# MGI-tech-bioinformatics/SuperPlus

Hardware: AMD Instinct MI355X
Metric: k-mers/s (DF createDict stage: trim + canonical k-mer count + solid filter + spectrum + adjacency) (higher is better)
Workload: dtype u64

## Files before the change

superplus_amd/csrc/dfk.hip:

```cpp
#include "../../include/dfk.h"
#include "dfk_kernels.h"

#include <algorithm>
#include <chrono>
#include <cstdarg>
#include <cstdio>
#include <cstdlib>
#include <cstring>
#include <atomic>
#include <fcntl.h>
#include <functional>
#include <new>
#include <string>
#include <sys/mman.h>
#include <sys/stat.h>
#include <unistd.h>
#include <condition_variable>
#include <memory>
#include <mutex>
#include <thread>
#include <vector>

using namespace dfk;

// ... 271 lines not shown
    float stop() { (void)hipEventRecord(b, s); (void)hipEventSynchronize(b); float ms = 0; (void)hipEventElapsedTime(&ms, a, b); return ms; }
};

uint32_t ceil_log2(uint64_t v) { uint32_t b = 0; while ((1ull << b) < v) ++b; return b; }

template <int K>
int stage_trim(dfk_ctx* c, const Inputs& in, uint64_t* n_inst)
{
    DevBuf ctr; int rc = c->alloc(ctr, 32, "trim counters"); if (rc) return rc;
    HIP_TRY(hipMemsetAsync(ctr.p, 0, 32, c->stream));
    rc = c->alloc(c->good_len, sizeof(uint32_t) * in.n_reads, "goodLens", true); if (rc) return rc;
    if (in.n_reads) {
        unsigned grid = (unsigned)std::min<uint64_t>((in.n_reads + 255) / 256, 8192);
        hipLaunchKernelGGL(HIP_KERNEL_NAME(k_trim<K>), dim3(grid), dim3(256), 0, c->stream,
                           in.pq, in.pq_off, in.pq_bytes, in.base_off, in.packed_bytes, in.read_len, in.n_reads, c->cfg.min_qual, (uint32_t*)c->good_len.p,
                           (unsigned long long*)ctr.p, (unsigned int*)((char*)ctr.p + 8),
                           (unsigned long long*)((char*)ctr.p + 16));
        HIP_TRY(hipGetLastError());
    }
    uint64_t h[3] = {0, 0, 0};
    HIP_TRY(hipMemcpyAsync(h, ctr.p, 24, hipMemcpyDeviceToHost, c->stream));
    HIP_TRY(hipStreamSynchronize(c->stream));
    c->release(ctr);
    if ((uint32_t)h[1]) return fail(DFK_E_INPUT, "malformed input: an offset table is not monotone or runs past its array, a PQVec stream is broken, or its length differs from read_len");
    if (h[2] == 0) return fail(DFK_E_NOGOOD, "Looks like your input data have almost no good bases.");
    *n_inst = h[0];
    return 0;
}

int device_scan(dfk_ctx* c, const uint64_t* in, uint64_t* out, uint64_t n)
{
    constexpr uint64_t PER = (uint64_t)SCAN_THREADS * SCAN_ITEMS;
    if (n == 0) return 0;
    const uint64_t nblk = (n + PER - 1) / PER;
    if (nblk == 1) {
        hipLaunchKernelGGL(k_scan_blocks, dim3(1), dim3(SCAN_THREADS), 0, c->stream, in, out, n, (uint64_t*)nullptr);
        HIP_TRY(hipGetLastError());
        return 0;
    }
    DevBuf sums; int rc = c->alloc(sums, nblk * 8, "scan block sums"); if (rc) return rc;
    hipLaunchKernelGGL(k_scan_blocks, dim3((unsigned)nblk), dim3(SCAN_THREADS), 0, c->stream, in, out, n, (uint64_t*)sums.p);
    HIP_TRY(hipGetLastError());
    rc = device_scan(c, (const uint64_t*)sums.p, (uint64_t*)sums.p, nblk); if (rc) return rc;
    hipLaunchKernelGGL(k_scan_add, dim3((unsigned)nblk), dim3(SCAN_THREADS), 0, c->stream, out, n, (const uint64_t*)sums.p);
    HIP_TRY(hipGetLastError());
    HIP_TRY(hipStreamSynchronize(c->stream));
    c->release(sums);
    return 0;
}

struct BucketTable {
    uint32_t log2_nb = 0;
    DevBuf acc;
    DevBuf summ;
    DevBuf classes;
    DevBuf ovf_list; uint64_t n_ovf = 0;
    DevBuf class_hist;
    std::vector<uint64_t> h_class;
    uint64_t n_records = 0, n_inst = 0;
};
struct Partition {
    DevBuf records, base, ipre, items;
    uint64_t n_records = 0, n_inst = 0, n_items = 0;
    uint64_t nb = 0;
};

template <int K>
PartParams part_params(const dfk_ctx* c, uint32_t log2_nb, uint32_t log2_world, int64_t read_id0, uint32_t sub_lo, uint32_t sub_n)
{
    const uint32_t M = c->cfg.minimizer_len;
    return PartParams{M, (uint32_t)K - M + 1, log2_nb, log2_world, read_id0, sub_lo, sub_n,
                      sweep_class_mask(sub_lo, sub_n, log2_nb - log2_world)};
}

int table_totals(dfk_ctx* c, const DevBuf& acc, uint64_t nb, uint64_t* n_records, uint64_t* n_inst)
{
    DevBuf tot; int rc = c->alloc(tot, 16, "bucket totals"); if (rc) return rc;
    HIP_TRY(hipMemsetAsync(tot.p, 0, 16, c->stream));
    hipLaunchKernelGGL(k_sum_acc, dim3(1024), dim3(256), 0, c->stream, (const unsigned long long*)acc.p, nb, (unsigned long long*)tot.p);
    HIP_TRY(hipGetLastError());
    uint64_t h[2];
    HIP_TRY(hipMemcpyAsync(h, tot.p, 16, hipMemcpyDeviceToHost, c->stream));
    HIP_TRY(hipStreamSynchronize(c->stream));
    c->release(tot);
    *n_records = h[0]; *n_inst = h[1];
    return 0;
}

struct ScanJob {
    PartParams pp; uint64_t nb = 0, n_bins = 0, ovf_cap = 0; bool by_class = false, ranged = false;
    DevBuf ovf_tmp, d_n;
    bool keyed = false; uint32_t n_cls = 0, n_sub = 0, sb = 0; uint64_t piece_reads = 0;
    ScanKeys sk{};
    DevBuf keys, keys2, fill, sub;
    std::vector<std::pair<hipEvent_t, hipEvent_t>> ev;
    ~ScanJob() { for (auto& e : ev) { (void)hipEventDestroy(e.first); (void)hipEventDestroy(e.second); } }
};

template <int K> bool scan_takes_ranges(const dfk_ctx* c) { return c->cfg.minimizer_len == 16; }

template <int K>
int scan_begin(dfk_ctx* c, const Inputs& in, uint32_t log2_world, int64_t read_id0, BucketTable* T, bool by_class, ScanJob* J)
{
    J->pp = part_params<K>(c, T->log2_nb, log2_world, read_id0, 0, 1u << (T->log2_nb - log2_world));
    J->nb = 1ull << T->log2_nb; J->by_class = by_class;
    int rc = 0;
    J->n_bins = 2ull * (PART_CLASSES << log2_world);
    if (by_class) { rc = c->alloc(T->class_hist, J->n_bins * 8, "class counters", true); if (rc) return rc; HIP_TRY(hipMemsetAsync(T->class_hist.p, 0, J->n_bins * 8, c->stream)); }
    else { rc = c->alloc(T->acc, J->nb * 8, "bucket counters", true); if (rc) return rc; }
    rc = c->alloc(T->summ, std::max<uint64_t>(1, in.n_reads) * 16, "run summaries", true); if (rc) return rc;
    rc = c->alloc(T->classes, std::max<uint64_t>(1, in.n_reads) * 4, "read bucket classes", true); if (rc) return rc;
    if (!by_class) HIP_TRY(hipMemsetAsync(T->acc.p, 0, J->nb * 8, c->stream));
    J->ovf_cap = in.n_reads / 16 + 1024;
    rc = c->alloc(J->ovf_tmp, J->ovf_cap * 4, "overflow read list (scratch)"); if (rc) return rc;
    rc = c->alloc(J->d_n, 16, "overflow read count"); if (rc) return rc;
    HIP_TRY(hipMemsetAsync(J->d_n.p, 0, 16, c->stream));
    const double runs = in.n_reads ? 1.0 + 2.0 * std::max(0.0, 4.0 * (double)in.packed_bytes / (double)in.n_reads - K + 1) / (J->pp.W + 1) : 0.0;
    J->keyed = !by_class && scan_takes_ranges<K>(c) && in.n_reads && (runs >= 3.5 || getenv("DFK_SCAN_KEY_PIECE"));
    if (J->keyed) {
        const uint32_t lb = T->log2_nb, cb = std::min<uint32_t>(6, lb);
        J->sk.ib = lb - cb; J->n_cls = 1u << cb;
        J->sb = std::min(KEY_SUB_BITS, J->sk.ib); J->n_sub = 1u << (J->sk.ib - J->sb);
        const double per_read = 1.25 * runs;
        constexpr uint64_t KEY_SCRATCH_MAX = 16ull << 30;
        const uint64_t want = 8ull * (uint64_t)(per_read * (double)in.n_reads) + 8ull * J->n_cls;
        const uint64_t room = std::min<uint64_t>(std::min(want, KEY_SCRATCH_MAX), c->largest_allocatable() / 3);
        J->sk.cap = std::max<uint64_t>(1024, room / 8 / J->n_cls);
        J->piece_reads = std::max<uint64_t>(PART_THREADS, (uint64_t)((double)(J->sk.cap * J->n_cls) / per_read));
        if (const char* e = getenv("DFK_SCAN_KEY_PIECE")) J->piece_reads = std::max<uint64_t>(1, std::min<uint64_t>(J->piece_reads, strtoull(e, nullptr, 10)));
        const uint64_t n_subs = (uint64_t)J->n_cls * J->n_sub;
        rc = c->alloc(J->keys, J->sk.cap * J->n_cls * 4, "run keys (scratch)"); if (rc) return rc;
        rc = c->alloc(J->keys2, J->sk.cap * J->n_cls * 4, "run keys by sub-slice (scratch)"); if (rc) return rc;
        rc = c->alloc(J->fill, J->n_cls * 8, "run key slice fills (scratch)"); if (rc) return rc;
        rc = c->alloc(J->sub, (3 * n_subs + 1) * 8, "run key sub-slices (scratch)"); if (rc) return rc;
        J->sk.keys = (uint32_t*)J->keys.p; J->sk.fill = (unsigned long long*)J->fill.p;
        TRACE("run keys: %u classes of %llu keys, %u sub-slices each, pieces of %llu reads", J->n_cls, (unsigned long long)J->sk.cap,
              J->n_sub, (unsigned long long)J->piece_reads);
    }
    return 0;
}

template <int K>
int scan_keys_piece(dfk_ctx* c, const Inputs& in, BucketTable* T, ScanJob* J, uint64_t r0, uint64_t r1)
{
    static const unsigned scan_blocks = getenv("DFK_SCAN_BLOCKS") ? (unsigned)atoi(getenv("DFK_SCAN_BLOCKS")) : 0;
    const unsigned cus = (unsigned)c->prop.multiProcessorCount;
    const unsigned grid = (unsigned)std::min<uint64_t>((r1 - r0 + PART_THREADS - 1) / PART_THREADS, (uint64_t)(scan_blocks ? scan_blocks : 128u) * cus);
    const uint64_t n_subs = (uint64_t)J->n_cls * J->n_sub;
    auto* cnt = (unsigned long long*)J->sub.p;
    auto* off = cnt + n_subs;
    auto* cur = off + n_subs + 1;
    HIP_TRY(hipMemsetAsync(J->fill.p, 0, J->n_cls * 8, c->stream));
    HIP_TRY(hipMemsetAsync(cnt, 0, n_subs * 8, c->stream));
    const size_t lds = sizeof(uint32_t) * (PART_RING + SUMMARY_RUNS) * PART_THREADS + SCAN_STAGE_LDS;
    hipLaunchKernelGGL(HIP_KERNEL_NAME(k_scan_count<K, 16, true>), dim3(grid), dim3(PART_THREADS), lds, c->stream,
                       in.packed, in.packed_bytes, in.base_off, (const uint32_t*)c->good_len.p, r0, r1, J->pp,
                       (unsigned long long*)T->acc.p, (unsigned long long*)nullptr, (unsigned long long*)J->d_n.p, J->ovf_cap,
                       (uint32_t*)J->ovf_tmp.p, (uint4*)T->summ.p, (uint32_t*)T->classes.p, J->sk);
    HIP_TRY(hipGetLastError());
    const dim3 per_class(std::max(1u, 16u * cus / J->n_cls), J->n_cls);
    const uint32_t sh = 6 + J->sb;
    hipLaunchKernelGGL(k_keys_subcount, per_class, dim3(256), J->n_sub * 4, c->stream,
                       (const uint32_t*)J->keys.p, (const unsigned long long*)J->fill.p, J->sk.cap, sh, J->n_sub, cnt);
    HIP_TRY(hipGetLastError());
    hipLaunchKernelGGL(k_keys_offsets, dim3(1), dim3(1024), 0, c->stream, (const unsigned long long*)cnt, (uint32_t)n_subs, off, cur);
    HIP_TRY(hipGetLastError());
    hipLaunchKernelGGL(k_keys_partition, per_class, dim3(256), J->n_sub * 12, c->stream,
                       (const uint32_t*)J->keys.p, (const unsigned long long*)J->fill.p, J->sk.cap, sh, J->n_sub, cur, (uint32_t*)J->keys2.p);
    HIP_TRY(hipGetLastError());
    hipLaunchKernelGGL(k_keys_count, dim3((unsigned)n_subs), dim3(1024), 0, c->stream,
                       (const uint32_t*)J->keys2.p, (const unsigned long long*)off, J->sb, (unsigned long long*)T->acc.p);
    HIP_TRY(hipGetLastError());
    return 0;
}

template <int K>
int scan_range(dfk_ctx* c, const Inputs& in, BucketTable* T, ScanJob* J, uint64_t r0, uint64_t r1)
{
    if (r1 <= r0) return 0;
    const PartParams& pp = J->pp;
    const bool by_class = J->by_class;
    unsigned grid = (unsigned)((r1 - r0 + PART_THREADS - 1) / PART_THREADS);
    static const unsigned scan_blocks = getenv("DFK_SCAN_BLOCKS") ? (unsigned)atoi(getenv("DFK_SCAN_BLOCKS")) : 0;
    if (by_class) grid = std::min<unsigned>(grid, (scan_blocks ? scan_blocks : 128u) * (unsigned)c->prop.multiProcessorCount);
    else if (scan_blocks) grid = std::min<unsigned>(grid, scan_blocks * (unsigned)c->prop.multiProcessorCount);
    const size_t lds_a = (sizeof(uint32_t) + 1) * pp.W * PART_THREADS + sizeof(uint32_t) * PART_RING * PART_THREADS + (by_class ? J->n_bins * 4 : 0);
    hipEvent_t e0, e1;
    HIP_TRY(hipEventCreate(&e0)); HIP_TRY(hipEventCreate(&e1));
    J->ev.emplace_back(e0, e1);
    HIP_TRY(hipEventRecord(e0, c->stream));
    if (J->keyed) {
        for (uint64_t p0 = r0; p0 < r1; p0 += J->piece_reads) {
            int rc = scan_keys_piece<K>(c, in, T, J, p0, std::min(r1, p0 + J->piece_reads)); if (rc) return rc;
        }
    } else if (scan_takes_ranges<K>(c)) {
        const size_t lds_r = sizeof(uint32_t) * (PART_RING + SUMMARY_RUNS) * PART_THREADS + (by_class ? J->n_bins * 4 : 0);
        hipLaunchKernelGGL(HIP_KERNEL_NAME(k_scan_count<K, 16, false>), dim3(grid), dim3(PART_THREADS), lds_r, c->stream,
                           in.packed, in.packed_bytes, in.base_off, (const uint32_t*)c->good_len.p, r0, r1, pp,
                           (unsigned long long*)T->acc.p, (unsigned long long*)T->class_hist.p, (unsigned long long*)J->d_n.p, J->ovf_cap,
                           (uint32_t*)J->ovf_tmp.p, (uint4*)T->summ.p, (uint32_t*)T->classes.p, ScanKeys{});
    } else {
        if (r0 != 0 || r1 != in.n_reads) return fail(DFK_E_STATE, "the general scan takes every read at once");
        hipLaunchKernelGGL(HIP_KERNEL_NAME(k_partition<K, false>), dim3(grid), dim3(PART_THREADS), lds_a, c->stream,
                           in.packed, in.packed_bytes, in.base_off, (const uint32_t*)c->good_len.p, in.bc,
                           (int64_t)c->cfg.ign_bc_below, in.n_reads, pp, (unsigned long long*)T->acc.p, (unsigned long long*)T->class_hist.p,
                           (unsigned long long*)J->d_n.p, J->ovf_cap, (uint4*)J->ovf_tmp.p, (uint4*)T->summ.p,
                           (const uint32_t*)nullptr, (uint64_t)0, (const uint64_t*)nullptr, (uint32_t*)T->classes.p);
    }
    HIP_TRY(hipGetLastError());
    HIP_TRY(hipEventRecord(e1, c->stream));
    return 0;
}

template <int K>
int scan_end(dfk_ctx* c, const Inputs& in, uint64_t n_inst, BucketTable* T, ScanJob* J)
{
    int rc = 0;
    T->n_ovf = 0;
    c->release(J->keys); c->release(J->keys2); c->release(J->fill); c->release(J->sub);
    if (in.n_reads) {
        HIP_TRY(hipMemcpyAsync(&T->n_ovf, J->d_n.p, 8, hipMemcpyDeviceToHost, c->stream));
        HIP_TRY(hipStreamSynchronize(c->stream));
        if (T->n_ovf > J->ovf_cap) {
            c->release(J->ovf_tmp);
            rc = c->alloc(J->ovf_tmp, in.n_reads * 4, "overflow read list (scratch)"); if (rc) return rc;
            HIP_TRY(hipMemsetAsync(J->d_n.p, 0, 16, c->stream));
            hipLaunchKernelGGL(k_select_overflow, dim3((unsigned)std::min<uint64_t>((in.n_reads + 255) / 256, 8192)), dim3(256), 0, c->stream,
                               (const uint4*)T->summ.p, in.n_reads, (uint32_t*)J->ovf_tmp.p, (unsigned long long*)J->d_n.p);
            HIP_TRY(hipGetLastError());
            HIP_TRY(hipMemcpyAsync(&T->n_ovf, J->d_n.p, 8, hipMemcpyDeviceToHost, c->stream));
            HIP_TRY(hipStreamSynchronize(c->stream));
        }
        if (T->n_ovf) {
            rc = c->alloc(T->ovf_list, T->n_ovf * 4, "overflow read list", true); if (rc) return rc;
            HIP_TRY(hipMemcpyAsync(T->ovf_list.p, J->ovf_tmp.p, T->n_ovf * 4, hipMemcpyDeviceToDevice, c->stream));
            HIP_TRY(hipStreamSynchronize(c->stream));
        }
    }
    c->release(J->ovf_tmp); c->release(J->d_n);
    HIP_TRY(hipStreamSynchronize(c->stream));
    float ms = 0;
    for (auto& e : J->ev) { float m = 0; if (hipEventElapsedTime(&m, e.first, e.second) == hipSuccess) ms += m; }
    c->st.ms_part_count = ms; c->st.reserved[6] = J->ev.size();
    TRACE("%llu of %llu reads have more than %d runs", (unsigned long long)T->n_ovf, (unsigned long long)in.n_reads, SUMMARY_RUNS);
    if (J->by_class) {
        T->h_class.assign(J->n_bins, 0);
        HIP_TRY(hipMemcpyAsync(T->h_class.data(), T->class_hist.p, J->n_bins * 8, hipMemcpyDeviceToHost, c->stream));
        HIP_TRY(hipStreamSynchronize(c->stream));
        T->n_records = T->n_inst = 0;
        for (uint64_t i = 0; i < J->n_bins / 2; ++i) { T->n_records += T->h_class[i]; T->n_inst += T->h_class[J->n_bins / 2 + i]; }
    } else { rc = table_totals(c, T->acc, J->nb, &T->n_records, &T->n_inst); if (rc) return rc; }
    TRACE("partition count pass done (%llu buckets, %llu records%s)", (unsigned long long)J->nb, (unsigned long long)T->n_records, J->ev.size() > 1 ? ", in ranges under the upload" : "");
    if (T->n_inst != n_inst)
        return fail(DFK_E_HIP, "partition count pass saw %llu instances, trim saw %llu%s",
                    (unsigned long long)T->n_inst, (unsigned long long)n_inst,
                    (n_inst - T->n_inst) % (1ull << 32) == 0 ? " (a fine bucket with 2^32 or more instances: its counter keeps 32 bits)" : "");
    c->st.n_records = T->n_records; c->st.n_buckets = J->nb;
    return 0;
}

template <int K>
int partition_count(dfk_ctx* c, const Inputs& in, uint64_t n_inst, uint32_t log2_world, int64_t read_id0, BucketTable* T, bool by_class = false)
{
    ScanJob J;
    int rc = scan_begin<K>(c, in, log2_world, read_id0, T, by_class, &J); if (rc) return rc;
    rc = scan_range<K>(c, in, T, &J, 0, in.n_reads); if (rc) return rc;
    return scan_end<K>(c, in, n_inst, T, &J);
}

int pass_tables(dfk_ctx* c, const DevBuf& acc, uint32_t log2_sub, uint32_t world, uint32_t sub_lo, uint32_t sub_n, uint64_t budget, Partition* P)
{
    P->nb = (uint64_t)world * sub_n;
    const uint64_t nb = P->nb;
    DevBuf rec, inst, flags, idx;
    int rc = c->alloc(rec, (nb + 1) * 8, "bucket record counts"); if (rc) return rc;
    rc = c->alloc(inst, (nb + 1) * 8, "bucket instance counts"); if (rc) return rc;
    rc = c->alloc(P->base, (nb + 1) * 8, "bucket bases"); if (rc) return rc;
    rc = c->alloc(P->ipre, (nb + 1) * 8, "bucket instance prefix"); if (rc) return rc;
    const unsigned g1 = (unsigned)((nb + 1 + 255) / 256);
    hipLaunchKernelGGL(k_slice, dim3(g1), dim3(256), 0, c->stream, (const unsigned long long*)acc.p, log2_sub, sub_lo, sub_n, nb,
                       (uint64_t*)rec.p, (uint64_t*)inst.p);
    HIP_TRY(hipGetLastError());
    rc = device_scan(c, (const uint64_t*)rec.p, (uint64_t*)P->base.p, nb + 1); if (rc) return rc;
    rc = device_scan(c, (const uint64_t*)inst.p, (uint64_t*)P->ipre.p, nb + 1); if (rc) return rc;
    rc = c->alloc(flags, (nb + 1) * 8, "item flags"); if (rc) return rc;
    rc = c->alloc(idx, (nb + 1) * 8, "item index"); if (rc) return rc;
    hipLaunchKernelGGL(k_item_flags, dim3(g1), dim3(256), 0, c->stream, (const uint64_t*)P->ipre.p, nb, budget, (uint64_t*)flags.p);
    HIP_TRY(hipGetLastError());
    rc = device_scan(c, (const uint64_t*)flags.p, (uint64_t*)idx.p, nb + 1); if (rc) return rc;
    uint64_t tot[3];
    HIP_TRY(hipMemcpyAsync(&tot[0], (const uint64_t*)P->base.p + nb, 8, hipMemcpyDeviceToHost, c->stream));
    HIP_TRY(hipMemcpyAsync(&tot[1], (const uint64_t*)P->ipre.p + nb, 8, hipMemcpyDeviceToHost, c->stream));
    HIP_TRY(hipMemcpyAsync(&tot[2], (const uint64_t*)idx.p + nb, 8, hipMemcpyDeviceToHost, c->stream));
    HIP_TRY(hipStreamSynchronize(c->stream));
    P->n_records = tot[0]; P->n_inst = tot[1]; P->n_items = tot[2];
    rc = c->alloc(P->items, std::max<uint64_t>(1, P->n_items) * sizeof(ItemRange), "work items"); if (rc) return rc;
    hipLaunchKernelGGL(k_item_pairs, dim3((unsigned)((nb + 255) / 256)), dim3(256), 0, c->stream, (const uint64_t*)flags.p,
                       (const uint64_t*)idx.p, nb, (ItemRange*)P->items.p);
    HIP_TRY(hipGetLastError());
    HIP_TRY(hipStreamSynchronize(c->stream));
    c->release(rec); c->release(inst); c->release(flags); c->release(idx);
    return 0;
}

void release_pass(dfk_ctx* c, Partition* P)
{ c->release(P->records); c->release(P->base); c->release(P->ipre); c->release(P->items); }

template <int K> uint64_t item_budget(const dfk_ctx* c)
{
    constexpr uint64_t S = 1ull << CountCfg<K>::LOG2S;
    if (c->cfg.inst_per_item) return c->cfg.inst_per_item;
    if (c->distinct_per_inst <= 0.0) return 3 * S / 2;
    const double b = 0.367 * (double)S / c->distinct_per_inst;
    return (uint64_t)std::min(std::max(b, 0.5 * (double)S), 3.0 * (double)S);
}

struct ScatterJob { Partition P; DevBuf cur, d_bad; hipStream_t st = nullptr; hipEvent_t e0 = nullptr, e1 = nullptr; uint32_t lo = 0, n = 0; };

template <int K>
int scatter_launch(dfk_ctx* c, const Inputs& in, const BucketTable& T, uint32_t log2_world, int64_t read_id0, ScatterJob* J)
{
    const PartParams pp = part_params<K>(c, T.log2_nb, log2_world, read_id0, J->lo, J->n);
    HIP_TRY(hipEventRecord(J->e0, J->st));
    if (in.n_reads)
        hipLaunchKernelGGL(HIP_KERNEL_NAME(k_scatter_runs<K>), dim3((unsigned)((in.n_reads + 256ull * sweep_reads<K>() - 1) / (256ull * sweep_reads<K>()))),
                           dim3(256), 0, J->st,
                           in.packed, in.packed_bytes, in.base_off, (const uint32_t*)c->good_len.p, in.bc,
                           (int64_t)c->cfg.ign_bc_below, in.n_reads, pp, (const uint4*)T.summ.p, (const uint32_t*)T.classes.p,
                           (unsigned long long*)J->cur.p, J->P.n_records, (uint4*)J->P.records.p);
    HIP_TRY(hipGetLastError());
    HIP_TRY(hipEventRecord(J->e1, J->st));
    return 0;
}

template <int K>
int scatter_begin(dfk_ctx* c, const Inputs& in, const BucketTable& T, uint32_t log2_world, int64_t read_id0,
                  uint32_t sub_lo, uint32_t sub_n, ScatterJob* J, bool launch_now = true)
{
    Partition* P = &J->P;
    J->st = c->stream; J->lo = sub_lo; J->n = sub_n;
    const PartParams pp = part_params<K>(c, T.log2_nb, log2_world, read_id0, sub_lo, sub_n);
    const uint64_t budget = item_budget<K>(c);
    int rc = pass_tables(c, T.acc, T.log2_nb - log2_world, 1u << log2_world, sub_lo, sub_n, budget, P); if (rc) return rc;
    const uint64_t nb = P->nb;
    rc = c->alloc(J->cur, nb * 8, "bucket cursors"); if (rc) return rc;
    rc = c->alloc(P->records, P->n_records * 32, "super-k-mer records"); if (rc) return rc;
    rc = c->alloc(J->d_bad, 16, "scatter check"); if (rc) return rc;
    HIP_TRY(hipMemcpyAsync(J->cur.p, P->base.p, nb * 8, hipMemcpyDeviceToDevice, c->stream));
    HIP_TRY(hipMemsetAsync(J->d_bad.p, 0, 16, c->stream));
// ... 1594 lines not shown
```

superplus_amd/csrc/dfk_kernels.h:

```cpp
#pragma once
#include <type_traits>
#include "dfk_device.h"

namespace dfk {

template <int K>
__global__ void __launch_bounds__(256)
k_trim(const uint8_t* __restrict__ pq, const uint64_t* __restrict__ pq_off, uint64_t pq_nbytes,
       const uint64_t* __restrict__ base_off, uint64_t packed_bytes, const uint32_t* __restrict__ read_len,
       uint64_t n_reads, uint32_t min_qual, uint32_t* __restrict__ good_len,
       unsigned long long* __restrict__ n_inst, unsigned int* __restrict__ bad,
       unsigned long long* __restrict__ sum_good)
{
    unsigned long long mine = 0, good = 0;
    bool any_bad = false;
    for (uint64_t r = (uint64_t)blockIdx.x * blockDim.x + threadIdx.x; r < n_reads; r += (uint64_t)gridDim.x * blockDim.x) {
        uint32_t gl = 0;
        uint64_t p = pq_off[r], end = pq_off[r + 1];
        uint32_t idx = 0, run = 0;
        const uint64_t b0 = base_off[r], b1 = base_off[r + 1];
        bool ok = p <= end && end <= pq_nbytes && b0 <= b1 && b1 <= packed_bytes && b1 - b0 >= ((uint64_t)read_len[r] + 3) / 4;
        if (!ok) end = p;
        while (p < end) {
            uint32_t nQs = pq[p];
// ... 195 lines not shown
    };
    uint32_t wbits, wnext = 0;
    if (!WRITE) { fill(); wbits = ring[(wi & (PART_RING - 1)) * PART_THREADS + tid]; }
    else { wbits = wi < n_words ? words[wi] : 0u; wnext = wi + 1 < n_words ? words[wi + 1] : 0u; }
    uint32_t wpos = (uint32_t)bit0 & 31u;
    uint32_t sfx_next = 0xFFFFFFFFu;

    auto close_run = [&]() {
        if (WRITE && cur_b == 0xFFFFFFFFu) return;
        if (!WRITE) {
            if (lh) { const uint32_t bin = class_bin(cur_b, pp); atomicAdd(&lh[bin], 1u); atomicAdd(&lh[(PART_CLASSES << pp.log2_world) + bin], cur_nk); }
            else atomicAdd(&bucket_acc[cur_b], (1ull << 32) | cur_nk);
            cmask |= 1u << sweep_class_of(cur_b & ((1u << log2_local) - 1u), log2_local);
            if (qn < (uint32_t)SUMMARY_RUNS) {
                const uint64_t fld = cur_nk | (cur_rel << 6);
                const uint32_t b = 8u + 12u * qn;
                if (b < 64u) { sum_lo |= fld << b; if (b > 52u) sum_hi |= fld >> (64u - b); }
                else sum_hi |= fld << (b - 64u);
            }
            ++qn;
        } else {
            if (qn == PART_QCAP) {
                for (uint32_t e = 0; e < qn; ++e) {
                    uint32_t a = queue[(2 * e) * PART_THREADS + tid], b = queue[(2 * e + 1) * PART_THREADS + tid];
                    const uint64_t dst = place(b);
                    if (dst != ~0ull) emit_record<K>(words, n_words, bit0, a & 0xFFFFu, a >> 16, b, gl, tag, dst, records);
                }
                qn = 0;
            }
            queue[(2 * qn) * PART_THREADS + tid] = cur_s0 | (cur_nk << 16);
            queue[(2 * qn + 1) * PART_THREADS + tid] = cur_b;
            ++qn;
        }
    };

    for (uint32_t j = 0; j < gl; ++j) {
        uint32_t b = (wbits >> wpos) & 3u;
        wpos += 2;
        if (wpos == 32) {
            wpos = 0; ++wi;
            if (!WRITE) { if (wi == filled_to) fill(); wbits = ring[(wi & (PART_RING - 1)) * PART_THREADS + tid]; }
            else { wbits = wnext; wnext = wi + 1 < n_words ? words[wi + 1] : 0u; }
        }
        f = ((f << 2) | b) & mmask;
        rc = (rc >> 2) | ((3u - b) << rsh);
        if (j + 1 < M) continue;
        uint32_t h = mmer_hash(f < rc ? f : rc);
        const bool newmin = bi == 0 || h < P;
        P = newmin ? h : P;
        if (!WRITE) Pi = newmin ? bi : Pi;
        const uint32_t t = j + 1 - M;
        if (t + 1 >= W) {
            uint32_t mv = P;
            bool older = false;
            if (bi != W - 1) { const uint32_t sfx = sfx_next; older = sfx < mv; mv = older ? sfx : mv; }
            const uint32_t s = t + 1 - W;
            uint32_t bucket = bucket_of(mv, pp);
            if (WRITE) bucket = pass_local(bucket, pp);
            const bool open = s == 0 || bucket != cur_b || cur_nk == (uint32_t)KTraits<K>::NK_MAX;
            if (open) {
                if (s != 0) close_run();
                cur_b = bucket; cur_s0 = s; cur_nk = 1;
                if (!WRITE) cur_rel = older ? (uint32_t)sidx[(bi + 1) * PART_THREADS + tid] - bi - 1u : W - 1u - bi + Pi;
            } else ++cur_nk;
        }
        arr[bi * PART_THREADS + tid] = h;
        if (++bi == W) {
            uint32_t run = h, ri = W - 1;
            if (!WRITE) sidx[(W - 1) * PART_THREADS + tid] = (uint8_t)(W - 1);
            for (int i0 = (int)W - 2; i0 >= 0; i0 -= 8) {
                uint32_t v[8];
#pragma unroll
                for (int k = 0; k < 8; ++k) v[k] = i0 - k >= 0 ? arr[(i0 - k) * PART_THREADS + tid] : 0u;
#pragma unroll
                for (int k = 0; k < 8; ++k) {
                    const int i = i0 - k;
                    if (i >= 0) {
                        const bool lt = v[k] < run;
                        run = lt ? v[k] : run;
                        arr[i * PART_THREADS + tid] = run;
                        if (!WRITE) { ri = lt ? (uint32_t)i : ri; sidx[i * PART_THREADS + tid] = (uint8_t)ri; }
                    }
                }
            }
            bi = 0;
        }
        if (bi + 1 < W) sfx_next = arr[(bi + 1) * PART_THREADS + tid];
    }
    close_run();
    if (!WRITE) {
        const uint64_t lo = sum_lo | (qn <= (uint32_t)SUMMARY_RUNS ? qn : SUMMARY_OVERFLOW), hi = sum_hi;
        summaries[r] = uint4{(uint32_t)lo, (uint32_t)(lo >> 32), (uint32_t)hi, (uint32_t)(hi >> 32)};
        if (read_classes) read_classes[r] = cmask;
        if (qn > (uint32_t)SUMMARY_RUNS && bucket_cur) {
            const unsigned long long at = atomicAdd(bucket_cur, 1ull);
            if (at < n_out) reinterpret_cast<uint32_t*>(records)[at] = (uint32_t)r;
        }
    }
    if (WRITE) {
        for (uint32_t e = 0; e < qn; ++e) {
            uint32_t a = queue[(2 * e) * PART_THREADS + tid], b = queue[(2 * e + 1) * PART_THREADS + tid];
            const uint64_t dst = place(b);
            if (dst != ~0ull) emit_record<K>(words, n_words, bit0, a & 0xFFFFu, a >> 16, b, gl, tag, dst, records);
        }
    }
}

template <int K, bool WRITE>
__global__ void __launch_bounds__(PART_THREADS)
k_partition(const uint8_t* __restrict__ packed, uint64_t packed_bytes, const uint64_t* __restrict__ base_off,
            const uint32_t* __restrict__ good_len, const int32_t* __restrict__ bc, int64_t ign_bc_below,
            uint64_t n_reads, PartParams pp,
            unsigned long long* __restrict__ bucket_acc,
            unsigned long long* __restrict__ class_hist,
            unsigned long long* __restrict__ bucket_cur,
            uint64_t n_out,
            uint4* __restrict__ records,
            uint4* __restrict__ summaries,
            const uint32_t* __restrict__ read_list,
            uint64_t n_list,
            const uint64_t* __restrict__ slice_base,
            uint32_t* __restrict__ read_classes)
{
    extern __shared__ uint32_t smem[];
    uint32_t* lh = nullptr;
    const uint32_t n_bins = 2u * (PART_CLASSES << pp.log2_world);
    if (!WRITE && class_hist) {
        lh = reinterpret_cast<uint32_t*>(reinterpret_cast<uint8_t*>(smem) + 5 * pp.W * PART_THREADS + 4 * PART_RING * PART_THREADS);
        for (uint32_t i = threadIdx.x; i < n_bins; i += PART_THREADS) lh[i] = 0;
        __syncthreads();
    }
    const uint64_t n_work = (WRITE && read_list) ? n_list : n_reads;
    for (uint64_t r0 = (uint64_t)blockIdx.x * PART_THREADS; r0 < n_work; r0 += (uint64_t)gridDim.x * PART_THREADS)
        partition_read<K, WRITE>(r0 + threadIdx.x, smem, lh, packed, packed_bytes, base_off, good_len, bc, ign_bc_below, n_reads, pp,
                                 bucket_acc, bucket_cur, n_out, records, summaries, read_list, n_list, slice_base, read_classes);
    if (lh) {
        __syncthreads();
        for (uint32_t i = threadIdx.x; i < n_bins; i += PART_THREADS) if (lh[i]) atomicAdd(&class_hist[i], (unsigned long long)lh[i]);
    }
}

template <int I, int N, class F>
__device__ __forceinline__ void static_for(F&& f)
{
    if constexpr (I < N) { f(std::integral_constant<int, I>{}); static_for<I + 1, N>(f); }
}

struct ScanKeys {
    uint32_t* keys;
    unsigned long long* fill;
    uint64_t cap;
    uint32_t ib;
};
constexpr int SCAN_STAGE = 1792;
constexpr uint32_t KEY_SUB_BITS = 14;
constexpr uint32_t KEY_TILE = 16384;

template <int K, int M, bool KEYS>
__global__ void __launch_bounds__(PART_THREADS)
k_scan_count(const uint8_t* __restrict__ packed, uint64_t packed_bytes, const uint64_t* __restrict__ base_off,
             const uint32_t* __restrict__ good_len, uint64_t r_first, uint64_t n_reads , PartParams pp,
             unsigned long long* __restrict__ bucket_acc, unsigned long long* __restrict__ class_hist,
             unsigned long long* __restrict__ ovf_count, uint64_t ovf_cap, uint32_t* __restrict__ ovf_list,
             uint4* __restrict__ summaries, uint32_t* __restrict__ read_classes, ScanKeys sk)
{
    constexpr int W = K - M + 1;
    constexpr uint32_t mmask = M == 16 ? 0xFFFFFFFFu : ((1u << (2 * M)) - 1u);
    constexpr uint32_t rsh = 2 * (M - 1);
    constexpr int RUNS = SUMMARY_RUNS;
    static_assert(KTraits<K>::NK_MAX < 64, "nk takes the key's six low bits");
    extern __shared__ uint32_t smem[];
    uint32_t* ring = smem;
    uint32_t* runb = smem + PART_RING * PART_THREADS;
    uint32_t* lh = nullptr;
    const uint32_t n_bins = 2u * (PART_CLASSES << pp.log2_world);
    if (class_hist) {
        lh = runb + RUNS * PART_THREADS;
        for (uint32_t i = threadIdx.x; i < n_bins; i += PART_THREADS) lh[i] = 0;
        __syncthreads();
    }
    const int tid = threadIdx.x;
    uint32_t* st_key = runb + RUNS * PART_THREADS;
    unsigned long long* st_base = reinterpret_cast<unsigned long long*>(st_key + SCAN_STAGE);
    uint32_t* st_h = reinterpret_cast<uint32_t*>(st_base + PART_CLASSES);
    uint32_t* st_n = st_h + PART_CLASSES;
    uint8_t* st_cls = reinterpret_cast<uint8_t*>(st_n + 1);
    const uint32_t n_cls = 1u << (pp.log2_nb - sk.ib);
    if constexpr (KEYS) {
        if (tid < PART_CLASSES) st_h[tid] = 0;
        if (tid == 0) *st_n = 0;
        __syncthreads();
    }
    auto flush = [&]() {
        const uint32_t n = *st_n;
        if (tid < (int)n_cls) { const uint32_t h = st_h[tid]; if (h) st_base[tid] = atomicAdd(&sk.fill[tid], (unsigned long long)h); st_h[tid] = 0; }
        __syncthreads();
        for (uint32_t j = tid; j < n; j += PART_THREADS) {
            const uint32_t key = st_key[j], cls = st_cls[j];
            const unsigned long long at = st_base[cls] + atomicAdd(&st_h[cls], 1u);
            if (at < sk.cap) sk.keys[cls * sk.cap + at] = key;
            else atomicAdd(&bucket_acc[(cls << sk.ib) | (key >> 6)], (1ull << 32) | (key & 63u));
        }
        __syncthreads();
        if (tid < (int)n_cls) st_h[tid] = 0;
        if (tid == 0) *st_n = 0;
        __syncthreads();
    };
    const uint32_t* words = reinterpret_cast<const uint32_t*>(packed);
    const uint64_t n_words = (packed_bytes + 3) >> 2;
    const uint32_t log2_local = pp.log2_nb - pp.log2_world;
    for (uint64_t r0 = r_first + (uint64_t)blockIdx.x * PART_THREADS; r0 < n_reads; r0 += (uint64_t)gridDim.x * PART_THREADS) {
        const uint64_t r = r0 + tid;
        const uint32_t gl = r < n_reads ? good_len[r] : 0;
        const bool live = gl >= (uint32_t)K + 1;
        uint32_t qn = 0, cmask = 0;
        uint64_t sum_lo = 0, sum_hi = 0;
        if (live) {
            const uint64_t bit0 = base_off[r] * 8;
            uint64_t wi = bit0 >> 5, filled_to = wi;
            auto fill = [&]() {
                uint32_t w[PART_RING];
#pragma unroll
                for (int k = 0; k < PART_RING; ++k) w[k] = filled_to + k < n_words ? words[filled_to + k] : 0u;
#pragma unroll
                for (int k = 0; k < PART_RING; ++k) ring[((filled_to + k) & (PART_RING - 1)) * PART_THREADS + tid] = w[k];
                filled_to += PART_RING;
            };
            fill();
            uint32_t wbits = ring[(wi & (PART_RING - 1)) * PART_THREADS + tid], wpos = (uint32_t)bit0 & 31u;
            auto next_base = [&]() -> uint32_t {
                const uint32_t b = (wbits >> wpos) & 3u;
                wpos += 2;
                if (wpos == 32) { wpos = 0; ++wi; if (wi == filled_to) fill(); wbits = ring[(wi & (PART_RING - 1)) * PART_THREADS + tid]; }
                return b;
            };
            uint32_t f = 0, rc = 0;
            for (int j = 0; j < M - 1; ++j) { const uint32_t b = next_base(); f = ((f << 2) | b) & mmask; rc = (rc >> 2) | ((3u - b) << rsh); }
            const uint32_t n_mmers = gl - M + 1;
            uint32_t arr[W], sidxw[(W + 3) / 4];
            auto sidx_get = [&](int i) -> uint32_t { return (sidxw[i >> 2] >> (8 * (i & 3))) & 255u; };
            auto sidx_set = [&](int i, uint32_t v) { const uint32_t sh = 8u * (uint32_t)(i & 3); sidxw[i >> 2] = (sidxw[i >> 2] & ~(255u << sh)) | (v << sh); };
#pragma unroll
            for (int i = 0; i < (W + 3) / 4; ++i) sidxw[i] = 0;
            uint32_t P = 0, Pi = 0;
            uint32_t cur_b = 0, cur_nk = 0, cur_rel = 0;
            auto close_run = [&]() {
                if (qn < (uint32_t)RUNS) {
                    runb[qn * PART_THREADS + tid] = cur_b;
                    const uint64_t fld = cur_nk | (cur_rel << 6);
                    const uint32_t b = 8u + 12u * qn;
                    if (b < 64u) { sum_lo |= fld << b; if (b > 52u) sum_hi |= fld >> (64u - b); } else sum_hi |= fld << (b - 64u);
                } else {
                    if (lh) { const uint32_t bin = class_bin(cur_b, pp); atomicAdd(&lh[bin], 1u); atomicAdd(&lh[(PART_CLASSES << pp.log2_world) + bin], cur_nk); }
                    else atomicAdd(&bucket_acc[cur_b], (1ull << 32) | cur_nk);
                    cmask |= 1u << sweep_class_of(cur_b & ((1u << log2_local) - 1u), log2_local);
                }
                ++qn;
            };
            for (uint32_t t0 = 0; t0 < n_mmers; t0 += W) {
                static_for<0, W>([&](auto bi_c) {
                    constexpr int bi = decltype(bi_c)::value;
                    if (t0 + (uint32_t)bi < n_mmers) {
                        const uint32_t b = next_base();
                        f = ((f << 2) | b) & mmask;
                        rc = (rc >> 2) | ((3u - b) << rsh);
                        const uint32_t h = mmer_hash(f < rc ? f : rc);
                        const bool newmin = bi == 0 || h < P;
                        P = newmin ? h : P;
                        Pi = newmin ? (uint32_t)bi : Pi;
                        const bool first = t0 == 0;
                        if (!first || bi == W - 1) {
                            uint32_t mv = P;
                            bool older = false;
                            if constexpr (bi != W - 1) { older = arr[bi + 1] < mv; mv = older ? arr[bi + 1] : mv; }
                            const uint32_t bucket = bucket_of(mv, pp);
                            const bool open = first || bucket != cur_b || cur_nk == (uint32_t)KTraits<K>::NK_MAX;
                            if (open) {
                                if (!first) close_run();
                                cur_b = bucket; cur_nk = 1;
                                cur_rel = (bi != W - 1 && older) ? sidx_get(bi + 1 < W ? bi + 1 : 0) - (uint32_t)bi - 1u : (uint32_t)(W - 1 - bi) + Pi;
                            } else ++cur_nk;
                        }
                        arr[bi] = h;
                        if (bi == W - 1) {
                            uint32_t run = h, ri = W - 1;
                            sidx_set(W - 1, W - 1);
                            static_for<0, W - 1>([&](auto j_c) {
                                constexpr int i = W - 2 - decltype(j_c)::value;
                                const bool lt = arr[i] < run; run = lt ? arr[i] : run; arr[i] = run; ri = lt ? (uint32_t)i : ri; sidx_set(i, ri);
                            });
                        }
                    }
                });
            }
            close_run();
        }
        const uint32_t mine = min(qn, (uint32_t)RUNS);
        for (uint32_t i = 0; KEYS ? __syncthreads_or(i < mine) != 0 : __ballot(i < mine) != 0ull; ++i) {
            const bool has = i < mine;
            uint32_t cb = 0, nk = 0;
            if (has) {
                cb = runb[i * PART_THREADS + tid];
                const uint32_t bfld = 8u + 12u * i;
                nk = (uint32_t)(bfld + 12 <= 64 ? sum_lo >> bfld : bfld >= 64 ? sum_hi >> (bfld - 64) : (sum_lo >> bfld) | (sum_hi << (64 - bfld))) & 63u;
                if constexpr (!KEYS) {
                    if (lh) { const uint32_t bin = class_bin(cb, pp); atomicAdd(&lh[bin], 1u); atomicAdd(&lh[(PART_CLASSES << pp.log2_world) + bin], nk); }
                    else atomicAdd(&bucket_acc[cb], (1ull << 32) | nk);
                }
                cmask |= 1u << sweep_class_of(cb & ((1u << log2_local) - 1u), log2_local);
            }
            if constexpr (KEYS) {
                const uint64_t m = __ballot(has);
                if (m) {
                    const uint32_t rk = __builtin_amdgcn_mbcnt_hi((uint32_t)(m >> 32), __builtin_amdgcn_mbcnt_lo((uint32_t)m, 0u));
                    const int lead = __ffsll((unsigned long long)m) - 1;
                    uint32_t at = 0;
                    if (has && rk == 0) at = atomicAdd(st_n, (uint32_t)__popcll(m));
                    at = __shfl(at, lead) + rk;
                    if (has) {
                        const uint32_t cls = cb >> sk.ib;
                        st_key[at] = ((cb & ((1u << sk.ib) - 1u)) << 6) | nk;
                        st_cls[at] = (uint8_t)cls;
                        atomicAdd(&st_h[cls], 1u);
                    }
                }
                __syncthreads();
                if (*st_n > (uint32_t)(SCAN_STAGE - PART_THREADS)) flush();
            }
        }
        if (r < n_reads) {
            const uint64_t lo = sum_lo | (qn <= (uint32_t)SUMMARY_RUNS ? qn : SUMMARY_OVERFLOW);
            summaries[r] = uint4{(uint32_t)lo, (uint32_t)(lo >> 32), (uint32_t)sum_hi, (uint32_t)(sum_hi >> 32)};
            if (read_classes) read_classes[r] = cmask;
        }
        if (qn > (uint32_t)SUMMARY_RUNS) {
            const unsigned long long at = atomicAdd(ovf_count, 1ull);
            if (at < ovf_cap) ovf_list[at] = (uint32_t)r;
        }
    }
    if constexpr (KEYS) { __syncthreads(); if (*st_n) flush(); }
    if (lh) {
        __syncthreads();
        for (uint32_t i = threadIdx.x; i < n_bins; i += PART_THREADS) if (lh[i]) atomicAdd(&class_hist[i], (unsigned long long)lh[i]);
    }
}
constexpr size_t SCAN_STAGE_LDS = (sizeof(uint32_t) + 1) * SCAN_STAGE + (sizeof(unsigned long long) + sizeof(uint32_t)) * PART_CLASSES + sizeof(uint32_t);

__global__ void __launch_bounds__(256)
k_keys_subcount(const uint32_t* __restrict__ keys, const unsigned long long* __restrict__ fill, uint64_t cap, uint32_t sh ,
                uint32_t n_sub, unsigned long long* __restrict__ sub_cnt)
{
    extern __shared__ uint32_t lh[];
    const uint32_t c = blockIdx.y;
    for (uint32_t i = threadIdx.x; i < n_sub; i += blockDim.x) lh[i] = 0;
    __syncthreads();
    const uint64_t n = min((uint64_t)fill[c], cap);
    const uint32_t* k = keys + c * cap;
    for (uint64_t i = (uint64_t)blockIdx.x * blockDim.x + threadIdx.x; i < n; i += (uint64_t)gridDim.x * blockDim.x) atomicAdd(&lh[k[i] >> sh], 1u);
    __syncthreads();
    for (uint32_t i = threadIdx.x; i < n_sub; i += blockDim.x) if (lh[i]) atomicAdd(&sub_cnt[(uint64_t)c * n_sub + i], (unsigned long long)lh[i]);
}

__global__ void __launch_bounds__(1024)
k_keys_offsets(const unsigned long long* __restrict__ cnt, uint32_t n, unsigned long long* __restrict__ off, unsigned long long* __restrict__ cur)
{
    __shared__ unsigned long long part[1024];
    const uint32_t tid = threadIdx.x, per = (n + 1023) / 1024;
    const uint32_t lo = min(n, tid * per), hi = min(n, lo + per);
    unsigned long long s = 0;
    for (uint32_t i = lo; i < hi; ++i) s += cnt[i];
    part[tid] = s;
    __syncthreads();
    for (uint32_t d = 1; d < 1024; d <<= 1) {
        const unsigned long long v = tid >= d ? part[tid - d] : 0ull;
        __syncthreads();
        part[tid] += v;
        __syncthreads();
    }
    unsigned long long run = part[tid] - s;
    for (uint32_t i = lo; i < hi; ++i) { off[i] = run; cur[i] = run; run += cnt[i]; }
    if (tid == 1023) off[n] = part[1023];
}

__global__ void __launch_bounds__(256)
k_keys_partition(const uint32_t* __restrict__ keys, const unsigned long long* __restrict__ fill, uint64_t cap, uint32_t sh,
                 uint32_t n_sub, unsigned long long* __restrict__ cur, uint32_t* __restrict__ out)
{
    extern __shared__ unsigned long long lds64[];
    unsigned long long* base = lds64;
    uint32_t* lh = reinterpret_cast<uint32_t*>(lds64 + n_sub);
    const uint32_t c = blockIdx.y;
    const uint64_t n = min((uint64_t)fill[c], cap);
    const uint32_t* k = keys + c * cap;
    unsigned long long* cc = cur + (uint64_t)c * n_sub;
    for (uint64_t t0 = (uint64_t)blockIdx.x * KEY_TILE; t0 < n; t0 += (uint64_t)gridDim.x * KEY_TILE) {
        const uint64_t t1 = min(n, t0 + KEY_TILE);
        for (uint32_t i = threadIdx.x; i < n_sub; i += blockDim.x) lh[i] = 0;
        __syncthreads();
        for (uint64_t i = t0 + threadIdx.x; i < t1; i += blockDim.x) atomicAdd(&lh[k[i] >> sh], 1u);
        __syncthreads();
        for (uint32_t i = threadIdx.x; i < n_sub; i += blockDim.x) { if (lh[i]) base[i] = atomicAdd(&cc[i], (unsigned long long)lh[i]); lh[i] = 0; }
        __syncthreads();
        for (uint64_t i = t0 + threadIdx.x; i < t1; i += blockDim.x) {
            const uint32_t key = k[i], s = key >> sh;
            out[base[s] + atomicAdd(&lh[s], 1u)] = key;
        }
        __syncthreads();
    }
}

__global__ void __launch_bounds__(1024)
k_keys_count(const uint32_t* __restrict__ part, const unsigned long long* __restrict__ off, uint32_t sb, unsigned long long* __restrict__ bucket_acc)
{
    __shared__ unsigned long long t[1u << KEY_SUB_BITS];
    const uint32_t s = blockIdx.x, nt = 1u << sb, m = nt - 1u;
    for (uint32_t i = threadIdx.x; i < nt; i += blockDim.x) t[i] = 0;
    __syncthreads();
    const uint64_t a = off[s], b = off[s + 1];
    for (uint64_t i = a + threadIdx.x; i < b; i += blockDim.x) {
        const uint32_t key = part[i];
        atomicAdd(&t[(key >> 6) & m], (1ull << 32) | (key & 63u));
    }
    __syncthreads();
    unsigned long long* dst = bucket_acc + ((uint64_t)s << sb);
    for (uint32_t i = threadIdx.x; i < nt; i += blockDim.x) if (t[i]) dst[i] += t[i];
}

constexpr int SLICE_READS = 16;
template <int K, bool EMIT, typename F>
__device__ __forceinline__ void for_each_run_in_pass(uint64_t r, const uint8_t* __restrict__ packed, uint64_t packed_bytes,
                                                     const uint64_t* __restrict__ base_off, const PartParams& pp,
                                                     const uint4* __restrict__ summaries, F&& f)
{
    const uint4 sm = summaries[r];
    const uint32_t n = sm.x & 15u;
    if (n == 0 || n == SUMMARY_OVERFLOW) return;
    const uint32_t* words = reinterpret_cast<const uint32_t*>(packed);
    const uint64_t n_words = (packed_bytes + 3) >> 2;
    const uint64_t bit0 = base_off[r] * 8;
    const uint32_t M = pp.M;
    const uint32_t mmask = M == 16 ? 0xFFFFFFFFu : ((1u << (2 * M)) - 1u);
    const uint64_t lo = (uint64_t)sm.x | ((uint64_t)sm.y << 32), hi = (uint64_t)sm.z | ((uint64_t)sm.w << 32);
    uint32_t s0 = 0;
#pragma unroll
    for (int i = 0; i < SUMMARY_RUNS; ++i) {
        if ((uint32_t)i < n) {
            constexpr int B0 = 8;
            const int b = B0 + 12 * i;
            const uint32_t fld = (uint32_t)(b + 12 <= 64 ? lo >> b : b >= 64 ? hi >> (b - 64) : (lo >> b) | (hi << (64 - b))) & 0xFFFu;
            const uint32_t nk = fld & 63u, rel = fld >> 6;
            const uint64_t bo = bit0 + 2ull * (s0 + rel);
            const uint64_t wi = bo >> 5;
            const uint32_t w0 = words[wi], w1 = wi + 1 < n_words ? words[wi + 1] : 0u;
            const uint32_t x = alignbit(w1, w0, (uint32_t)bo & 31u) & mmask;
            uint32_t y = __brev(x);
            y = ((y >> 1) & 0x55555555u) | ((y & 0x55555555u) << 1);
            const uint32_t fw = y >> (32 - 2 * M), rcv = ~x & mmask;
            const uint32_t bucket = bucket_of(mmer_hash(fw < rcv ? fw : rcv), pp);
            const uint32_t lb = pass_local(bucket, pp);
            if (lb != 0xFFFFFFFFu) f(s0, nk, lb, bucket >> (pp.log2_nb - pp.log2_world), bit0, (uint32_t)i + 1 == n);
            s0 += nk;
        }
    }
}

template <int K>
__global__ void __launch_bounds__(256)
k_scatter_slices(const uint8_t* __restrict__ packed, uint64_t packed_bytes, const uint64_t* __restrict__ base_off,
                 const uint32_t* __restrict__ good_len, const int32_t* __restrict__ bc, int64_t ign_bc_below,
                 uint64_t n_reads, PartParams pp, const uint4* __restrict__ summaries, const uint32_t* __restrict__ read_classes,
                 const uint64_t* __restrict__ slice_base,
                 unsigned long long* __restrict__ slice_fill,
                 uint4* __restrict__ records)
{
    __shared__ uint32_t cnt[256];
    __shared__ unsigned long long at[256];
    __shared__ uint16_t list[256 * SLICE_READS];
    __shared__ uint32_t n_list;
    const uint32_t world = 1u << pp.log2_world;
    const int lane = threadIdx.x & 63;
    const uint64_t r_block = (uint64_t)blockIdx.x * 256 * SLICE_READS;
    if (threadIdx.x < world) cnt[threadIdx.x] = 0;
    if (threadIdx.x == 0) n_list = 0;
    __syncthreads();
#pragma unroll
    for (int j = 0; j < SLICE_READS; ++j) {
        const uint32_t rel = 256u * j + threadIdx.x;
        const uint64_t r = r_block + rel;
        const bool hit = r < n_reads && (!read_classes || (read_classes[r] & pp.class_mask) != 0u);
        const unsigned long long mk = __ballot(hit);
        uint32_t w = 0;
        if (lane == 0 && mk) w = atomicAdd(&n_list, (uint32_t)__popcll(mk));
        w = __builtin_amdgcn_readfirstlane(w);
        if (hit) list[w + __popcll(mk & ((1ull << lane) - 1ull))] = (uint16_t)rel;
    }
    __syncthreads();
    const uint32_t n = n_list;
    for (uint32_t i = threadIdx.x; i < n; i += 256)
        for_each_run_in_pass<K, false>(r_block + list[i], packed, packed_bytes, base_off, pp, summaries,
// ... 1551 lines not shown
```

Baseline: 60.31 billion.

## Replace LDS word ring with register window loads in the k-mer scan

```diff
diff --git a/superplus_amd/csrc/dfk.hip b/superplus_amd/csrc/dfk.hip
--- a/superplus_amd/csrc/dfk.hip
+++ b/superplus_amd/csrc/dfk.hip
@@ -447,7 +447,7 @@
     auto* cur = off + n_subs + 1;
     HIP_TRY(hipMemsetAsync(J->fill.p, 0, J->n_cls * 8, c->stream));
     HIP_TRY(hipMemsetAsync(cnt, 0, n_subs * 8, c->stream));
-    const size_t lds = sizeof(uint32_t) * (PART_RING + SUMMARY_RUNS) * PART_THREADS + SCAN_STAGE_LDS;
+    const size_t lds = SCAN_RUN_LDS + SCAN_STAGE_LDS;
     hipLaunchKernelGGL(HIP_KERNEL_NAME(k_scan_count<K, 16, true>), dim3(grid), dim3(PART_THREADS), lds, c->stream,
                        in.packed, in.packed_bytes, in.base_off, (const uint32_t*)c->good_len.p, r0, r1, J->pp,
                        (unsigned long long*)T->acc.p, (unsigned long long*)nullptr, (unsigned long long*)J->d_n.p, J->ovf_cap,
@@ -489,7 +489,7 @@
             int rc = scan_keys_piece<K>(c, in, T, J, p0, std::min(r1, p0 + J->piece_reads)); if (rc) return rc;
         }
     } else if (scan_takes_ranges<K>(c)) {
-        const size_t lds_r = sizeof(uint32_t) * (PART_RING + SUMMARY_RUNS) * PART_THREADS + (by_class ? J->n_bins * 4 : 0);
+        const size_t lds_r = SCAN_RUN_LDS + (by_class ? J->n_bins * 4 : 0);
         hipLaunchKernelGGL(HIP_KERNEL_NAME(k_scan_count<K, 16, false>), dim3(grid), dim3(PART_THREADS), lds_r, c->stream,
                            in.packed, in.packed_bytes, in.base_off, (const uint32_t*)c->good_len.p, r0, r1, pp,
                            (unsigned long long*)T->acc.p, (unsigned long long*)T->class_hist.p, (unsigned long long*)J->d_n.p, J->ovf_cap,
diff --git a/superplus_amd/csrc/dfk_kernels.h b/superplus_amd/csrc/dfk_kernels.h
--- a/superplus_amd/csrc/dfk_kernels.h
+++ b/superplus_amd/csrc/dfk_kernels.h
@@ -371,7 +371,7 @@
     uint64_t cap;
     uint32_t ib;
 };
-constexpr int SCAN_STAGE = 1792;
+constexpr int SCAN_STAGE = 1536;
 constexpr uint32_t KEY_SUB_BITS = 14;
 constexpr uint32_t KEY_TILE = 16384;
 
@@ -389,17 +389,18 @@
     constexpr int RUNS = SUMMARY_RUNS;
     static_assert(KTraits<K>::NK_MAX < 64, "nk takes the key's six low bits");
     extern __shared__ uint32_t smem[];
-    uint32_t* ring = smem;
-    uint32_t* runb = smem + PART_RING * PART_THREADS;
+    uint32_t* runb = smem;
+    uint16_t* runf = reinterpret_cast<uint16_t*>(runb + RUNS * PART_THREADS);
+    uint32_t* const after_runs = reinterpret_cast<uint32_t*>(runf + RUNS * PART_THREADS);
     uint32_t* lh = nullptr;
     const uint32_t n_bins = 2u * (PART_CLASSES << pp.log2_world);
     if (class_hist) {
-        lh = runb + RUNS * PART_THREADS;
+        lh = after_runs;
         for (uint32_t i = threadIdx.x; i < n_bins; i += PART_THREADS) lh[i] = 0;
         __syncthreads();
     }
     const int tid = threadIdx.x;
-    uint32_t* st_key = runb + RUNS * PART_THREADS;
+    uint32_t* st_key = after_runs;
     unsigned long long* st_base = reinterpret_cast<unsigned long long*>(st_key + SCAN_STAGE);
     uint32_t* st_h = reinterpret_cast<uint32_t*>(st_base + PART_CLASSES);
     uint32_t* st_n = st_h + PART_CLASSES;
@@ -436,25 +437,27 @@
         uint64_t sum_lo = 0, sum_hi = 0;
         if (live) {
             const uint64_t bit0 = base_off[r] * 8;
-            uint64_t wi = bit0 >> 5, filled_to = wi;
-            auto fill = [&]() {
-                uint32_t w[PART_RING];
-#pragma unroll
-                for (int k = 0; k < PART_RING; ++k) w[k] = filled_to + k < n_words ? words[filled_to + k] : 0u;
-#pragma unroll
-                for (int k = 0; k < PART_RING; ++k) ring[((filled_to + k) & (PART_RING - 1)) * PART_THREADS + tid] = w[k];
-                filled_to += PART_RING;
+            constexpr int NW = (2 * W + 30 + 31) / 32, NA = (2 * W + 31) / 32;
+            auto load = [&](uint64_t bit, uint32_t (&w)[NW]) {
+                const uint64_t wi = bit >> 5;
+#pragma unroll
+                for (int k = 0; k < NW; ++k) {
+                    const uint64_t i = wi + k;
+                    const uint32_t v = words[i < n_words ? i : n_words - 1];
+                    w[k] = i < n_words ? v : 0u;
+                }
             };
-            fill();
-            uint32_t wbits = ring[(wi & (PART_RING - 1)) * PART_THREADS + tid], wpos = (uint32_t)bit0 & 31u;
-            auto next_base = [&]() -> uint32_t {
-                const uint32_t b = (wbits >> wpos) & 3u;
-                wpos += 2;
-                if (wpos == 32) { wpos = 0; ++wi; if (wi == filled_to) fill(); wbits = ring[(wi & (PART_RING - 1)) * PART_THREADS + tid]; }
-                return b;
-            };
+            uint64_t nbit = bit0 + 2 * (M - 1);
+            uint32_t nw[NW];
+            load(nbit, nw);
             uint32_t f = 0, rc = 0;
-            for (int j = 0; j < M - 1; ++j) { const uint32_t b = next_base(); f = ((f << 2) | b) & mmask; rc = (rc >> 2) | ((3u - b) << rsh); }
+            {
+                const uint64_t wi = bit0 >> 5;
+                const uint32_t w0 = words[wi < n_words ? wi : n_words - 1], w1 = words[wi + 1 < n_words ? wi + 1 : n_words - 1];
+                const uint32_t pw = alignbit(wi + 1 < n_words ? w1 : 0u, wi < n_words ? w0 : 0u, (uint32_t)bit0 & 31u);
+#pragma unroll
+                for (int j = 0; j < M - 1; ++j) { const uint32_t b = (pw >> (2 * j)) & 3u; f = ((f << 2) | b) & mmask; rc = (rc >> 2) | ((3u - b) << rsh); }
+            }
             const uint32_t n_mmers = gl - M + 1;
             uint32_t arr[W], sidxw[(W + 3) / 4];
             auto sidx_get = [&](int i) -> uint32_t { return (sidxw[i >> 2] >> (8 * (i & 3))) & 255u; };
@@ -466,9 +469,7 @@
             auto close_run = [&]() {
                 if (qn < (uint32_t)RUNS) {
                     runb[qn * PART_THREADS + tid] = cur_b;
-                    const uint64_t fld = cur_nk | (cur_rel << 6);
-                    const uint32_t b = 8u + 12u * qn;
-                    if (b < 64u) { sum_lo |= fld << b; if (b > 52u) sum_hi |= fld >> (64u - b); } else sum_hi |= fld << (b - 64u);
+                    runf[qn * PART_THREADS + tid] = (uint16_t)(cur_nk | (cur_rel << 6));
                 } else {
                     if (lh) { const uint32_t bin = class_bin(cur_b, pp); atomicAdd(&lh[bin], 1u); atomicAdd(&lh[(PART_CLASSES << pp.log2_world) + bin], cur_nk); }
                     else atomicAdd(&bucket_acc[cur_b], (1ull << 32) | cur_nk);
@@ -477,10 +478,18 @@
                 ++qn;
             };
             for (uint32_t t0 = 0; t0 < n_mmers; t0 += W) {
+                uint32_t a[NA];
+                {
+                    const uint32_t sh = (uint32_t)nbit & 31u;
+#pragma unroll
+                    for (int i = 0; i < NA; ++i) a[i] = alignbit(i + 1 < NW ? nw[i + 1] : 0u, nw[i], sh);
+                }
+                nbit += 2 * W;
+                load(nbit, nw);
                 static_for<0, W>([&](auto bi_c) {
                     constexpr int bi = decltype(bi_c)::value;
                     if (t0 + (uint32_t)bi < n_mmers) {
-                        const uint32_t b = next_base();
+                        const uint32_t b = (a[(2 * bi) >> 5] >> ((2 * bi) & 31)) & 3u;
                         f = ((f << 2) | b) & mmask;
                         rc = (rc >> 2) | ((3u - b) << rsh);
                         const uint32_t h = mmer_hash(f < rc ? f : rc);
@@ -494,11 +503,11 @@
                             if constexpr (bi != W - 1) { older = arr[bi + 1] < mv; mv = older ? arr[bi + 1] : mv; }
                             const uint32_t bucket = bucket_of(mv, pp);
                             const bool open = first || bucket != cur_b || cur_nk == (uint32_t)KTraits<K>::NK_MAX;
-                            if (open) {
-                                if (!first) close_run();
-                                cur_b = bucket; cur_nk = 1;
-                                cur_rel = (bi != W - 1 && older) ? sidx_get(bi + 1 < W ? bi + 1 : 0) - (uint32_t)bi - 1u : (uint32_t)(W - 1 - bi) + Pi;
-                            } else ++cur_nk;
+                            if (open && !first) close_run();
+                            const uint32_t rel = (bi != W - 1 && older) ? sidx_get(bi + 1 < W ? bi + 1 : 0) - (uint32_t)bi - 1u : (uint32_t)(W - 1 - bi) + Pi;
+                            cur_rel = open ? rel : cur_rel;
+                            cur_nk = open ? 1u : cur_nk + 1u;
+                            cur_b = open ? bucket : cur_b;
                         }
                         arr[bi] = h;
                         if (bi == W - 1) {
@@ -520,8 +529,10 @@
             uint32_t cb = 0, nk = 0;
             if (has) {
                 cb = runb[i * PART_THREADS + tid];
+                const uint64_t fld = runf[i * PART_THREADS + tid];
+                nk = (uint32_t)fld & 63u;
                 const uint32_t bfld = 8u + 12u * i;
-                nk = (uint32_t)(bfld + 12 <= 64 ? sum_lo >> bfld : bfld >= 64 ? sum_hi >> (bfld - 64) : (sum_lo >> bfld) | (sum_hi << (64 - bfld))) & 63u;
+                if (bfld < 64u) { sum_lo |= fld << bfld; if (bfld > 52u) sum_hi |= fld >> (64u - bfld); } else sum_hi |= fld << (bfld - 64u);
                 if constexpr (!KEYS) {
                     if (lh) { const uint32_t bin = class_bin(cb, pp); atomicAdd(&lh[bin], 1u); atomicAdd(&lh[(PART_CLASSES << pp.log2_world) + bin], nk); }
                     else atomicAdd(&bucket_acc[cb], (1ull << 32) | nk);
@@ -563,7 +574,9 @@
         for (uint32_t i = threadIdx.x; i < n_bins; i += PART_THREADS) if (lh[i]) atomicAdd(&class_hist[i], (unsigned long long)lh[i]);
     }
 }
+constexpr size_t SCAN_RUN_LDS = (sizeof(uint32_t) + sizeof(uint16_t)) * SUMMARY_RUNS * PART_THREADS;
 constexpr size_t SCAN_STAGE_LDS = (sizeof(uint32_t) + 1) * SCAN_STAGE + (sizeof(unsigned long long) + sizeof(uint32_t)) * PART_CLASSES + sizeof(uint32_t);
+static_assert(SCAN_RUN_LDS + SCAN_STAGE_LDS <= 16384, "ten scan blocks a CU (160 KB of LDS)");
 
 __global__ void __launch_bounds__(256)
 k_keys_subcount(const uint32_t* __restrict__ keys, const unsigned long long* __restrict__ fill, uint64_t cap, uint32_t sh ,
```

New measurement: 61.96 billion, median of 6. 2.7% higher.
